# ljishen/bitar

Measured on AMD Instinct MI355X. Metric: GiB/s compress+decompress on 1-GiB Arrow buffer, 1/2/4/8 GPUs; % HBM roofline, higher is better.
Workload: dtype u8; 1 GPU; LZ4 block compress + decompress round trip, 1 GiB per GPU, 64 KiB segments, Silesia-style mix (BASELINE configs[2]); bytes_per_gpu=1073741824, segment_bytes=65536, segments_per_gpu=16384, codec=lz4-block, input_kind=1, parallelism=1 GPU

## Files before the change

### bitar_amd/csrc/compress.hip

```cpp
#include "window_parse.hip.h"

namespace bitar_hip {

namespace cmp {

__device__ __forceinline__ uint32_t lane_sel(uint64_t m, uint32_t a, uint32_t b) {
  uint32_t r;
  __asm__("v_cndmask_b32_e64 %0, %1, %2, %3" : "=v"(r) : "v"(b), "v"(a), "s"(m));
  return r;
}

#ifndef BITAR_LZ4_GATHER
#define BITAR_LZ4_GATHER 3
#endif
#ifndef BITAR_LZ4_OBUF
#define BITAR_LZ4_OBUF 512
#endif
constexpr uint32_t kLz4Obuf = BITAR_LZ4_OBUF;
constexpr uint32_t kSeqCap = 64;
struct Lz4Lds {
#if BITAR_LZ4_GATHER == 3
  uint8_t ring[kLz4Obuf + 16];
#elif BITAR_LZ4_GATHER == 2
  uint8_t ring[kLz4Obuf];
#else
  uint8_t ring[kLz4Obuf + kWave];
#endif
  uint2 seqs[kSeqCap + 1];
  uint32_t marks[kWave + 1];
};

struct Lz4Out : ByteOutT<kLz4Obuf> {
  Lz4Lds* L;
  uint32_t nseq;
  uint32_t last_end;
  uint32_t step_id;

  __device__ __forceinline__ void init(Lz4Lds* lds, GMEM uint8_t* d, uint64_t c) {
    L = lds;
    ring = lds->ring;
    dst = d;
    cap = c;
    op = flushed = 0;
    overflow = false;
    nseq = 0;
    last_end = 0;
    step_id = 0;
    lds->marks[lane_id()] = 0;
    lds_order();
  }
  __device__ __forceinline__ void put_ext(uint32_t v) {
    const uint32_t cnt = v / 255u + 1;
    for (uint32_t k = 0; k < cnt; k += kWave) {
      const uint32_t step = cnt - k < kWave ? cnt - k : kWave;
      if (!room(step)) return;
      const uint32_t t = k + lane_id();
      put(t + 1 < cnt ? 255u : v % 255u, step);
    }
  }
  __device__ __forceinline__ void one(const GMEM uint8_t* in, const InRing& I, uint32_t lit_start,
                                      uint32_t lit_len, uint32_t off, uint32_t mlen) {
    if (overflow) return;
    const uint32_t ml = mlen ? mlen - kMinMatch : 0;
    const uint32_t token = ((lit_len < 15 ? lit_len : 15) << 4) | (ml < 15 ? ml : 15);
    if (!room(1)) return;
    put(token, 1);
    if (lit_len >= 15) put_ext(lit_len - 15);
    if (overflow) return;
    if (lit_len) {
      if ((uint64_t)op + lit_len > cap) { overflow = true; return; }
      if (lit_len <= 256 && lit_start >= I.lo) {
        for (uint32_t k = 0; k < lit_len; k += kWave) {
          const uint32_t step = lit_len - k < kWave ? lit_len - k : kWave;
          room(step);
          lds_order();
          const uint32_t b = I.byte(lit_start + k + (lane_id() < step ? lane_id() : 0u));
          put(b, step);
        }
      } else {
        flush(op, true);
        wave_copy_global(dst + op, in + lit_start, lit_len);
        op += lit_len;
        flushed = op;
      }
    }
    if (!mlen) return;
    if (!room(2)) return;
    put(lane_id() ? off >> 8 : off & 0xFF, 2);
    if (ml >= 15) put_ext(ml - 15);
  }

#if BITAR_LZ4_GATHER == 3
  __device__ __forceinline__ bool bulk(const InRing& I, uint32_t lo, uint32_t hi, uint32_t q,
                                       uint32_t lit_start, uint32_t off, uint32_t mlen) {
    constexpr uint32_t kTrash = kLz4Obuf, kLim = kLz4Obuf - 64;
    const uint32_t lane = lane_id();
    const bool in = (lane >= lo) & (lane < hi);
    const uint32_t lit_len = q - lit_start, ml = mlen - kMinMatch;
    const uint32_t nlx = lit_len >= 15 ? 1u : 0u, nmx = ml >= 15 ? 1u : 0u;
    const uint32_t e = in ? (3u + nlx + nmx + lit_len) | (lit_len << 16) : 0u;
    const uint32_t incl = wave_incl_sum(e);
    const uint32_t total = readlane(incl, kWave - 1) & 0xFFFFu;
// ... 95 lines not shown
      if (op + kWave - flushed > kLz4Obuf - 64) flush(op, false);
      lds_order();
      const uint32_t slot = min(a4 - (R << 2), (uint32_t)kWave << 2);
      *reinterpret_cast<uint32_t*>(reinterpret_cast<uint8_t*>(L->marks) + slot) = mark;
      lds_order();
      const uint32_t mk = L->marks[lane];
      L->marks[lane] = zero;
      const uint64_t S = ballot(mk == u);
      const uint32_t base = before + (uint32_t)(S & 1u);
      const uint64_t S1 = S >> 1;
      const uint32_t idx = __builtin_amdgcn_mbcnt_hi((uint32_t)(S1 >> 32),
                                                     __builtin_amdgcn_mbcnt_lo((uint32_t)S1, 0u));
      before += (uint32_t)__builtin_popcountll(S);
      const int src = (int)((idx << 2) + (base << 2));
      const uint32_t qA = (uint32_t)__builtin_amdgcn_ds_bpermute(src, (int)pA);
      const uint32_t qH = (uint32_t)__builtin_amdgcn_ds_bpermute(src, (int)pH);
      const uint32_t qT = (uint32_t)__builtin_amdgcn_ds_bpermute(src, (int)pT);
      const uint32_t r = u - (qA & 0xFFFFu);
      const uint32_t t = u - (qA >> 16);
      const uint32_t sel = min(min(t, r + 4u), 6u);
      const uint32_t litb = I.ring[(((u << 16) + qH) >> 16) & I.mask];
      const uint32_t hi4 = __builtin_amdgcn_perm(litb, qH, 0x0C040100u);
      const uint32_t b = __builtin_amdgcn_perm(hi4, qT, sel);
      const uint32_t nb = total - R < kWave ? total - R : kWave;
      ring[(rbase + u) & kMask] = (uint8_t)b;
      lds_order();
      op += nb;
      u += kWave;
    }
    return true;
  }
#else
  __device__ __forceinline__ bool bulk(const InRing& I, uint32_t lo, uint32_t hi, uint32_t q,
                                       uint32_t lit_start, uint32_t off, uint32_t mlen) {
    const uint32_t lane = lane_id();
    const bool in = (lane >= lo) & (lane < hi);
    const uint32_t lit_len = q - lit_start, ml = mlen - kMinMatch;
    const uint32_t nlx = lit_len >= 15 ? 1u : 0u, nmx = ml >= 15 ? 1u : 0u;
    const uint32_t e = in ? 3u + nlx + nmx + lit_len : 0u;
    const uint32_t incl = wave_incl_sum(e);
    const uint32_t total = readlane(incl, kWave - 1);
    if ((uint64_t)op + total > cap) return false;
    const uint32_t a = incl - e;
    const uint32_t tok = ((lit_len < 15 ? lit_len : 15) << 4) | (ml < 15 ? ml : 15);
    const uint32_t p0 = a | (lit_len << 16) | (nlx << 25) | (nmx << 26);
    const uint32_t p1 = lit_start | (tok << 16);
    const uint32_t p2 = (off & 0xFFFFu) | (((ml - 15u) & 0xFFu) << 16) | ((lit_len - 15u) << 24);
    for (uint32_t R = 0; R < total; R += kWave) {
      room(kWave);
      step_id += 1;
      const bool st = in & (a - R < kWave);
      lds_order();
      L->marks[st ? a - R : kWave] = (step_id << 8) | (lane + 1);
      lds_order();
      const uint32_t mk = L->marks[lane];
      const uint32_t before = (uint32_t)__builtin_popcountll(ballot(in & (a < R)));
      const uint32_t carry = before ? lo + before : 0u;
      const uint32_t v = (mk >> 8) == step_id ? (mk & 0xFFu) : 0u;
      const uint32_t s1 = max(wave_incl_max(v), carry);
      const int src = (int)((s1 - 1) << 2);
      const uint32_t q0 = (uint32_t)__builtin_amdgcn_ds_bpermute(src, (int)p0);
      const uint32_t q1 = (uint32_t)__builtin_amdgcn_ds_bpermute(src, (int)p1);
      const uint32_t q2 = (uint32_t)__builtin_amdgcn_ds_bpermute(src, (int)p2);
      const uint32_t r = R + lane - (q0 & 0xFFFFu);
      const uint32_t ll = (q0 >> 16) & 511u;
      const uint32_t L0 = 1u + ((q0 >> 25) & 1u), h = L0 + ll;
      const uint32_t litb = I.byte((q1 & 0xFFFFu) + r - L0);
      uint32_t b = r == h + 2 ? (q2 >> 16) & 0xFFu : (q2 >> 8) & 0xFFu;
      b = r == h ? q2 & 0xFFu : b;
      b = r < h ? litb : b;
      b = r < L0 ? q2 >> 24 : b;
      b = r == 0 ? (q1 >> 16) & 0xFFu : b;
      const uint32_t nb = total - R < kWave ? total - R : kWave;
      lds_order();
      ring[lane < nb ? at(op + lane) : kLz4Obuf + lane] = (uint8_t)b;
      lds_order();
      op += nb;
    }
    return true;
  }
#endif

  __device__ __forceinline__ void flush_seqs(const GMEM uint8_t* in, const InRing& I) {
    const uint32_t cnt = nseq;
    nseq = 0;
    if (!cnt || overflow) return;
    const uint32_t lane = lane_id();
    lds_order();
    const uint2 rec = L->seqs[lane < cnt ? lane : kSeqCap];
    const uint32_t q = rec.x & 0xFFFFu, off = (rec.x >> 16) + 1u, mlen = rec.y;
    const uint32_t end = q + mlen;
    const uint32_t prev = wave_shr1(end);
    const uint32_t lit_start = lane == 0 ? last_end : prev;
    const uint32_t lit_len = q - lit_start;
    last_end = readlane(end, cnt - 1);
    const uint64_t live = cnt < kWave ? (1ull << cnt) - 1 : ~0ull;
    uint64_t special = (ballot(lit_len >= 270u) | ballot(mlen >= 270u + kMinMatch) |
                        ballot(lit_start < I.lo)) & live;
    uint32_t lo = 0;
    for (;;) {
      const uint32_t k = special ? (uint32_t)__builtin_ctzll(special) : cnt;
      if (k > lo && !bulk(I, lo, k, q, lit_start, off, mlen)) {
        for (uint32_t j = lo; j < k && !overflow; ++j)
          one(in, I, readlane(lit_start, j), readlane(lit_len, j), readlane(off, j),
              readlane(mlen, j));
      }
      if (k >= cnt || overflow) break;
      one(in, I, readlane(lit_start, k), readlane(lit_len, k), readlane(off, k),
          readlane(mlen, k));
      special &= special - 1;
      lo = k + 1;
    }
  }

  __device__ __forceinline__ void sequence(const GMEM uint8_t* in, const InRing& I,
                                           uint32_t lit_start, uint32_t lit_len, uint32_t off,
                                           uint32_t mlen) {
    flush_seqs(in, I);
    one(in, I, lit_start, lit_len, off, mlen);
  }
  __device__ __forceinline__ uint32_t pending_from(uint32_t anchor, uint32_t) const { return anchor; }

  __device__ __forceinline__ void between(const GMEM uint8_t* in, const InRing& I) {
    if (BITAR_RARE(nseq > kSeqCap - 16)) flush_seqs(in, I);
  }
  __device__ __forceinline__ void window(const GMEM uint8_t*, const InRing&, const Window& W,
                                         uint32_t, uint32_t) {
    if (!W.chain) return;
    const uint64_t chain = W.chain;
    const uint32_t idx = __builtin_amdgcn_mbcnt_hi((uint32_t)(chain >> 32),
                                                   __builtin_amdgcn_mbcnt_lo((uint32_t)chain, nseq));
    const uint32_t lane = lane_id();
    lds_order();
    L->seqs[lane_sel(chain, idx, kSeqCap)] =
        make_uint2((W.x + lane) | (W.dm1 << 16), W.mlen);
    lds_order();
    nseq += (uint32_t)__builtin_popcountll(chain);
  }
};

constexpr uint32_t kBitWords = BITAR_CMP_BITWORDS, kBitMask = kBitWords - 1;

__device__ __forceinline__ uint32_t rev(uint32_t v, uint32_t n) {
  return __builtin_bitreverse32(v) >> (32 - n);
}
__device__ __forceinline__ uint32_t fixed_code(uint32_t s, uint32_t& n) {
  const uint32_t code = s < 144 ? 0x30 + s : s < 256 ? 0x190 + (s - 144) : s < 280 ? s - 256 : 0xC0 + (s - 280);
  n = s < 144 ? 8u : s < 256 ? 9u : s < 280 ? 7u : 8u;
  return __builtin_bitreverse32(code) >> (32 - n);
}
__device__ __forceinline__ uint32_t match_code(uint32_t mlen, uint32_t off, uint32_t& n) {
  const uint32_t v = mlen - 3;
  const uint32_t lev = 29u - __builtin_clz(v | 8u);
  const uint32_t le = mlen == 258 || v < 8 ? 0u : lev;
  const uint32_t lc = mlen == 258 ? 28u : v < 8 ? v : 4 * lev + 4 + ((v >> lev) & 3u);
  const uint32_t lx = v & ((1u << le) - 1);
  const uint32_t d = off - 1;
  const uint32_t dev = 30u - __builtin_clz(d | 4u);
  const uint32_t de = d < 4 ? 0u : dev;
  const uint32_t dc = d < 4 ? d : 2 * dev + 2 + ((d >> dev) & 1u);
  const uint32_t dx = d & ((1u << de) - 1);
  uint32_t ln;
  const uint32_t code = fixed_code(257 + lc, ln);
  n = ln + le + 5 + de;
  return code | (lx << ln) | (rev(dc, 5) << (ln + le)) | (dx << (ln + le + 5));
}

#ifndef BITAR_DFL_BULK
#define BITAR_DFL_BULK 1
#endif
struct DflLds {
  uint2 recs[kSeqCap + 1];
  uint32_t marks[kWave + 1];
};
struct DflOut {
  uint32_t* stage;
  GMEM uint32_t* dst;
  uint64_t cap;
  uint64_t bits;
  uint32_t wflushed;
  bool overflow;

  __device__ __forceinline__ void flush_words(uint32_t upto) {
    const uint32_t lane = lane_id();
    lds_order();
    for (uint32_t w = wflushed + lane; w < upto; w += kWave) {
      dst[w] = stage[w & kBitMask];
      stage[w & kBitMask] = 0;
    }
    lds_order();
    wflushed = upto;
  }
  __device__ __forceinline__ void drain() {
    const uint32_t full = (uint32_t)(bits >> 5);
    if (full != wflushed) flush_words(full);
  }
  __device__ __forceinline__ void put_lanes(uint32_t val, uint32_t nb) {
    if (overflow) return;
    const uint32_t incl = wave_incl_sum(nb);
    const uint32_t total = readlane(incl, 63);
    if ((bits + total + 7) / 8 > cap) { overflow = true; return; }
    const uint64_t bp = bits + incl - nb;
    const uint32_t w = (uint32_t)(bp >> 5), sh = (uint32_t)(bp & 31);
    const uint32_t spill = sh + nb > 32 ? val >> ((32 - sh) & 31) : 0u;
    lds_order();
    if (nb) atomicOr(&stage[w & kBitMask], val << sh);
    if (sh + nb > 32) atomicOr(&stage[(w + 1) & kBitMask], spill);
    lds_order();
    bits += total;
    const uint32_t full = (uint32_t)(bits >> 5);
    if (full - wflushed >= kBitWords - 80) flush_words(full);
  }
  __device__ __forceinline__ void put_one(uint32_t val, uint32_t nb) {
    put_lanes(lane_id() == 0 ? val : 0u, lane_id() == 0 ? nb : 0u);
  }
  __device__ __forceinline__ void literals(const GMEM uint8_t* in, const InRing& I, uint32_t s,
                                           uint32_t n) {
    const uint32_t lane = lane_id();
    const bool ring_ok = s >= I.lo;
    for (uint32_t k = 0; k < n; k += kWave) {
      const uint32_t step = n - k < kWave ? n - k : kWave;
      const uint32_t q = s + k + (lane < step ? lane : 0);
      uint32_t b;
      lds_order();
      if (ring_ok) b = I.byte(q);
      else b = lane < step ? (uint32_t)in[q] : 0u;
      uint32_t nb;
      const uint32_t code = fixed_code(b, nb);
      put_lanes(lane < step ? code : 0u, lane < step ? nb : 0u);
      if (overflow) return;
    }
  }
#if BITAR_DFL_BULK
  DflLds* L;
  uint32_t npend, last_end;

  __device__ __forceinline__ void bulk(const InRing& I, uint32_t lo, uint32_t hi,
                                       uint32_t lit_start, uint32_t ll, uint32_t mv, uint32_t mb) {
    const uint32_t lane = lane_id();
    const bool in = (lane >= lo) & (lane < hi);
    const uint32_t e = in ? ll + 1u : 0u;
    const uint32_t incl = wave_incl_sum(e);
    const uint32_t total = readlane(incl, kWave - 1);
    const uint32_t a = incl - e;
    const uint32_t D = I.in_lo + lit_start - a - 1u;
    const uint32_t pX = ((a + ll + 1u) << 16) | mb;
    const uint32_t a4 = in ? a << 2 : 0x7FFFFF00u;
    const uint32_t mark = a + 1u;
    const uint32_t zero = 0;
    uint32_t u = lane + 1u;
    uint32_t before = lo - 1u;
    for (uint32_t R = 0; R < total && !overflow; R += kWave) {
      lds_order();
      const uint32_t slot = min(a4 - (R << 2), (uint32_t)kWave << 2);
      *reinterpret_cast<uint32_t*>(reinterpret_cast<uint8_t*>(L->marks) + slot) = mark;
      lds_order();
      const uint32_t mk = L->marks[lane];
      L->marks[lane] = zero;
      const uint64_t S = ballot(mk == u);
      const uint32_t base = before + (uint32_t)(S & 1u);
      const uint64_t S1 = S >> 1;
      const uint32_t k = __builtin_amdgcn_mbcnt_hi((uint32_t)(S1 >> 32),
                                                   __builtin_amdgcn_mbcnt_lo((uint32_t)S1, 0u));
      before += (uint32_t)__builtin_popcountll(S);
      const int src = (int)((k << 2) + (base << 2));
      const uint32_t qD = (uint32_t)__builtin_amdgcn_ds_bpermute(src, (int)D);
      const uint32_t qX = (uint32_t)__builtin_amdgcn_ds_bpermute(src, (int)pX);
      const uint32_t qM = (uint32_t)__builtin_amdgcn_ds_bpermute(src, (int)mv);
      const uint32_t b = I.ring[(qD + u) & I.mask];
      uint32_t lb;
      const uint32_t lv = fixed_code(b, lb);
      const bool ism = u == (qX >> 16);
      const bool live = u <= total;
      put_lanes(ism ? qM : lv, live ? (ism ? (qX & 63u) : lb) : 0u);
      u += kWave;
    }
  }
  __device__ __forceinline__ void flush_seqs(const GMEM uint8_t* in, const InRing& I) {
    const uint32_t cnt = npend;
    npend = 0;
    if (!cnt || overflow) return;
    const uint32_t lane = lane_id();
    lds_order();
    const uint2 rec = L->recs[lane < cnt ? lane : kSeqCap];
    const uint32_t q = rec.x & 0xFFFFu, off = (rec.x >> 16) + 1u, mlen = rec.y;
    const uint32_t end = q + mlen;
    const uint32_t prev = wave_shr1(end);
    const uint32_t lit_start = lane == 0 ? last_end : prev;
    const uint32_t ll = q - lit_start;
    last_end = readlane(end, cnt - 1);
    uint32_t mb;
    const uint32_t mv = match_code(lane < cnt ? mlen : 3u, lane < cnt ? off : 1u, mb);
    const uint64_t live = cnt < kWave ? (1ull << cnt) - 1 : ~0ull;
    uint64_t special = ballot(lit_start < I.lo) & ballot(ll != 0u) & live;
    uint32_t lo = 0;
    for (;;) {
      const uint32_t k = special ? (uint32_t)__builtin_ctzll(special) : cnt;
      if (k > lo) bulk(I, lo, k, lit_start, ll, mv, mb);
      if (k >= cnt || overflow) break;
      literals(in, I, readlane(lit_start, k), readlane(ll, k));
      put_one(readlane(mv, k), readlane(mb, k));
      special &= special - 1;
      lo = k + 1;
    }
  }
  __device__ __forceinline__ uint32_t pending_from(uint32_t anchor, uint32_t) const { return anchor; }
  __device__ __forceinline__ void between(const GMEM uint8_t* in, const InRing& I) {
    if (BITAR_RARE(npend > kSeqCap - 16)) flush_seqs(in, I);
  }
  __device__ __forceinline__ void sequence(const GMEM uint8_t* in, const InRing& I, uint32_t s,
                                           uint32_t n, uint32_t, uint32_t) {
    flush_seqs(in, I);
    literals(in, I, s, n);
  }
  __device__ __forceinline__ void window(const GMEM uint8_t*, const InRing&, const Window& W,
// ... 173 lines not shown
```

### bitar_amd/csrc/deflate_dyn.hip

```cpp
#include "huffman.hip.h"
#include "window_parse.hip.h"

namespace bitar_hip {

namespace dyn {

using namespace cmp;

#ifndef BITAR_DYN_VARIANT
#define BITAR_DYN_VARIANT 0
#endif

constexpr uint32_t kPlanBytes = 2048;
constexpr uint32_t kNLit = 286, kNDist = 30, kNCl = 19;
constexpr uint32_t kPlanRecBytes = kNLit + kNDist;

__device__ __forceinline__ uint32_t len_sym(uint32_t mlen, uint32_t& nx, uint32_t& xv) {
  const uint32_t v = mlen - 3;
  const uint32_t lev = 29u - __builtin_clz(v | 8u);
  nx = mlen == 258 || v < 8 ? 0u : lev;
  xv = v & ((1u << nx) - 1);
  return mlen == 258 ? 28u : v < 8 ? v : 4 * lev + 4 + ((v >> lev) & 3u);
}
__device__ __forceinline__ uint32_t dist_sym(uint32_t off, uint32_t& nx, uint32_t& xv) {
// ... 3 lines not shown
  xv = d & ((1u << nx) - 1);
  return d < 4 ? d : 2 * dev + 2 + ((d >> dev) & 1u);
}
__device__ __forceinline__ uint32_t len_extra_bits(uint32_t ls) {
  return ls < 8 || ls == 28 ? 0u : (ls - 4) >> 2;
}
__device__ __forceinline__ uint32_t dist_extra_bits(uint32_t ds) {
  return ds < 4 ? 0u : (ds - 2) >> 1;
}
__constant__ uint8_t kClo[19] = {16, 17, 18, 0, 8, 7, 9, 6, 10, 5, 11, 4, 12, 3, 13, 2, 14, 1, 15};

__device__ __forceinline__ uint32_t fixed_len(uint32_t s) {
  return s < 144 ? 8u : s < 256 ? 9u : s < 280 ? 7u : 8u;
}

[[maybe_unused]] constexpr uint32_t kMaskBytes = 16384;
constexpr uint32_t kPlanWindows = kPlanRecBytes + 1;
constexpr uint32_t kPlanTail = kPlanRecBytes + 2;

constexpr uint32_t kRecBuf = 512, kMaskRing = 32;
struct RecOut : ByteOutT<kRecBuf> {
  uint32_t* lh;
  uint32_t* dh;
  uint4* cst;
  GMEM uint4* cdst;
  uint32_t nwin, cflushed;

  __device__ __forceinline__ void window(const GMEM uint8_t*, const InRing&, const Window& W,
                                         uint32_t, uint32_t n) {
    const uint32_t lane = lane_id();
    const uint32_t q = W.x + lane;
    const bool cl = (W.chain >> lane) & 1;
    const uint32_t pend = wave_incl_max(cl ? q + W.mlen : 0u);
    const bool covered = q < W.pos_in || (!cl && q < pend);
    const bool lit = !cl && !covered && q < n;
    const uint64_t litm = ballot(lit);
    uint32_t lnx, lxv, dnx, dxv;
    const uint32_t ls = len_sym(cl ? W.mlen : 3u, lnx, lxv);
    const uint32_t ds = dist_sym(cl ? W.off() : 1u, dnx, dxv);
    lds_order();
    if (lit) atomicAdd(&lh[W.byte], 1u);
    if (cl) {
      atomicAdd(&lh[257 + ls], 1u);
      atomicAdd(&dh[ds], 1u);
    }
    if (lane == 0)
      cst[nwin & (kMaskRing - 1)] = make_uint4((uint32_t)W.chain, (uint32_t)(W.chain >> 32), (uint32_t)litm,
                                   (uint32_t)(litm >> 32));
    lds_order();
    ++nwin;
    if (overflow || !W.chain) return;
    const uint32_t nm = (uint32_t)__builtin_popcountll(W.chain);
    if (!room(4 * nm)) return;
    const uint32_t rank = (uint32_t)__builtin_popcountll(W.chain & ((1ull << lane) - 1));
    uint32_t* r32 = reinterpret_cast<uint32_t*>(ring);
    lds_order();
    if (cl) r32[at(op + 4 * rank) >> 2] = ls | (lxv << 5) | (ds << 10) | (dxv << 15);
    lds_order();
    op += 4 * nm;
  }
  __device__ __forceinline__ void flush_masks(uint32_t upto) {
    const uint32_t lane = lane_id();
    lds_order();
    for (uint32_t w = cflushed + lane; w < upto; w += kWave) cdst[w] = cst[w & (kMaskRing - 1)];
    cflushed = upto;
  }
  __device__ __forceinline__ void drain() {
    ByteOutT<kRecBuf>::drain();
    flush_masks(nwin);
  }
  __device__ __forceinline__ void sequence(const GMEM uint8_t* in, const InRing& I, uint32_t s,
                                           uint32_t n, uint32_t, uint32_t) {
    const uint32_t lane = lane_id();
    const bool ring_ok = s >= I.lo;
    for (uint32_t k = 0; k < n; k += kWave) {
      const uint32_t step = n - k < kWave ? n - k : kWave;
      const uint32_t q = s + k + (lane < step ? lane : 0);
      lds_order();
      const uint32_t b = ring_ok ? I.byte(q) : (uint32_t)in[q];
      if (lane < step) atomicAdd(&lh[b], 1u);
      lds_order();
    }
  }
  __device__ __forceinline__ void between(const GMEM uint8_t*, const InRing&) {}
  __device__ __forceinline__ uint32_t pending_from(uint32_t, uint32_t emitted) const { return emitted; }
};

#ifndef BITAR_DYN_BULK
#define BITAR_DYN_BULK 1
#endif
#if BITAR_DYN_BULK
constexpr uint32_t kDynCap = 64;
#ifndef BITAR_DYN_OBUF
#define BITAR_DYN_OBUF 512
#endif
constexpr uint32_t kDynObuf = BITAR_DYN_OBUF;
constexpr uint32_t kDynGap = 1024;
__host__ __device__ constexpr uint32_t lit_cap(uint32_t seg) { return (seg + 15u) & ~15u; }
struct DynLds {
  uint8_t ring[kDynObuf];
  uint2 recs[kDynCap + 1];
  uint32_t marks[kWave + 1];
};
struct DynCollect : ByteOutT<kDynObuf> {
  DynLds* L;
  uint32_t* lh;
  uint32_t* dh;
  GMEM uint2* seqs;
  uint32_t nseq, rec_cap, npend;
  uint32_t last_end;
  uint32_t x_seen;

  __device__ __forceinline__ void lit_run(const GMEM uint8_t* in, const InRing& I, uint32_t s,
                                          uint32_t len) {
    const uint32_t lane = lane_id();
    for (uint32_t k = 0; k < len && !overflow; k += kWave) {
      const uint32_t step = len - k < kWave ? len - k : kWave;
      if (!room(step)) return;
      const uint32_t q = s + k + (lane < step ? lane : 0u);
      lds_order();
      const uint32_t b = s + k >= I.lo ? I.byte(q) : (uint32_t)in[q];
      if (lane < step) atomicAdd(&lh[b], 1u);
      put(b, step);
    }
  }
  __device__ __forceinline__ void gather(const InRing& I, uint32_t lo, uint32_t hi,
                                         uint32_t lit_start, uint32_t ll) {
    const uint32_t lane = lane_id();
    const bool ne = (lane >= lo) & (lane < hi) & (ll != 0u);
    const uint32_t e = ne ? ll : 0u;
    const uint32_t incl = wave_incl_sum(e);
    const uint32_t total = readlane(incl, kWave - 1);
    if (!total) return;
    if ((uint64_t)op + total > cap) { overflow = true; return; }
    const uint32_t a = incl - e;
    const uint64_t nem = ballot(ne);
    const uint32_t rank = __builtin_amdgcn_mbcnt_hi((uint32_t)(nem >> 32),
                                                    __builtin_amdgcn_mbcnt_lo((uint32_t)nem, 0u));
    const uint32_t D = I.in_lo + lit_start - a - 1u;
    lds_order();
    uint32_t* tmp = reinterpret_cast<uint32_t*>(L->recs);
    tmp[ne ? rank : kWave] = D;
    lds_order();
    const uint32_t Dc = tmp[lane];
    const uint32_t a4 = ne ? a << 2 : 0x7FFFFF00u;
    const uint32_t mark = a + 1u;
    const uint32_t zero = 0;
    const uint32_t rbase = (uint32_t)(uintptr_t)dst + op - 1u;
    uint32_t u = lane + 1u;
    uint32_t before = 0;
    lds_order();
    for (uint32_t R = 0; R < total; R += kWave) {
      if (op + kWave - flushed > kDynObuf - 64) flush(op, false);
      lds_order();
      const uint32_t slot = min(a4 - (R << 2), (uint32_t)kWave << 2);
      *reinterpret_cast<uint32_t*>(reinterpret_cast<uint8_t*>(L->marks) + slot) = mark;
      lds_order();
      const uint32_t mk = L->marks[lane];
      L->marks[lane] = zero;
      const uint64_t S = ballot(mk == u);
      const uint32_t base = before - 1u + (uint32_t)(S & 1u);
      const uint64_t S1 = S >> 1;
      const uint32_t k = __builtin_amdgcn_mbcnt_hi((uint32_t)(S1 >> 32),
                                                   __builtin_amdgcn_mbcnt_lo((uint32_t)S1, 0u));
      before += (uint32_t)__builtin_popcountll(S);
      const uint32_t d = (uint32_t)__builtin_amdgcn_ds_bpermute((int)((k << 2) + (base << 2)),
                                                                (int)Dc);
      const uint32_t b = I.ring[(d + u) & I.mask];
      const uint32_t nb = total - R < kWave ? total - R : kWave;
      if (lane < nb) atomicAdd(&lh[b], 1u);
      ring[(rbase + u) & kMask] = (uint8_t)b;
      lds_order();
      op += nb;
      u += kWave;
    }
  }
  __device__ __forceinline__ void flush_seqs(const GMEM uint8_t* in, const InRing& I) {
    const uint32_t cnt = npend;
    npend = 0;
    if (overflow) return;
    const uint32_t lane = lane_id();
    if (cnt) {
      lds_order();
      const uint2 rec = L->recs[lane < cnt ? lane : kDynCap];
      const uint32_t q = rec.x & 0xFFFFu, off = (rec.x >> 16) + 1u, mlen = rec.y;
      const uint32_t end = q + mlen;
      const uint32_t prev = wave_shr1(end);
      const uint32_t lit_start = lane == 0 ? last_end : prev;
      const uint32_t ll = q - lit_start;
      last_end = readlane(end, cnt - 1);
      if (nseq + cnt > rec_cap) { overflow = true; return; }
      if (lane < cnt) seqs[nseq + lane] = rec;
      nseq += cnt;
      uint32_t lnx, lxv, dnx, dxv;
      const uint32_t ls = len_sym(lane < cnt ? mlen : 3u, lnx, lxv);
      const uint32_t ds = dist_sym(lane < cnt ? off : 1u, dnx, dxv);
      lds_order();
      if (lane < cnt) {
        atomicAdd(&lh[257 + ls], 1u);
        atomicAdd(&dh[ds], 1u);
      }
      lds_order();
      const uint64_t live = cnt < kWave ? (1ull << cnt) - 1 : ~0ull;
      uint64_t special = ballot(lit_start < I.lo) & ballot(ll != 0u) & live;
      uint32_t lo = 0;
      for (;;) {
        const uint32_t k = special ? (uint32_t)__builtin_ctzll(special) : cnt;
        if (k > lo) gather(I, lo, k, lit_start, ll);
        if (k >= cnt || overflow) break;
        lit_run(in, I, readlane(lit_start, k), readlane(ll, k));
        special &= special - 1;
        lo = k + 1;
      }
    }
    if (x_seen > last_end && !overflow) {
      lit_run(in, I, last_end, x_seen - last_end);
      last_end = x_seen;
    }
  }
  __device__ __forceinline__ void between(const GMEM uint8_t* in, const InRing& I) {
    if (npend > kDynCap - 16 || x_seen > last_end + kDynGap) flush_seqs(in, I);
  }
  __device__ __forceinline__ void sequence(const GMEM uint8_t* in, const InRing& I, uint32_t s,
                                           uint32_t len, uint32_t, uint32_t) {
    x_seen = s + len;
    flush_seqs(in, I);
  }
  __device__ __forceinline__ uint32_t pending_from(uint32_t anchor, uint32_t) const { return anchor; }
  __device__ __forceinline__ void window(const GMEM uint8_t*, const InRing&, const Window& W,
                                         uint32_t, uint32_t n) {
    x_seen = W.x + kWave < n ? W.x + kWave : n;
    if (!W.chain) return;
    const uint64_t chain = W.chain;
    const uint32_t lane = lane_id();
    const uint32_t rank = __builtin_amdgcn_mbcnt_hi((uint32_t)(chain >> 32),
                                                    __builtin_amdgcn_mbcnt_lo((uint32_t)chain, 0u));
    lds_order();
    L->recs[(chain >> lane) & 1u ? npend + rank : kDynCap] =
        make_uint2((W.x + lane) | (W.dm1 << 16), W.mlen);
    lds_order();
    npend += (uint32_t)__builtin_popcountll(chain);
  }
};
#endif

using huf::TreeLds;
using huf::huff_lengths;

__device__ void canon_codes(const uint8_t* lens, uint32_t n, uint32_t* tab) {
  const uint32_t lane = lane_id();
  const uint64_t lt = (1ull << lane) - 1;
  uint32_t cnt[16];
#pragma unroll
  for (int b = 0; b < 16; ++b) cnt[b] = 0;
  lds_order();
  for (uint32_t s0 = 0; s0 < n; s0 += kWave) {
    const uint32_t s = s0 + lane;
    const uint32_t l = s < n ? lens[s] : 0u;
#pragma unroll
    for (int b = 1; b < 16; ++b) cnt[b] += (uint32_t)__builtin_popcountll(ballot(l == (uint32_t)b));
  }
  uint32_t first[16];
  uint32_t code = 0;
  first[0] = 0;
#pragma unroll
  for (int b = 1; b < 16; ++b) {
    code = (code + (b > 1 ? cnt[b - 1] : 0u)) << 1;
    first[b] = code;
    cnt[b - 1] = 0;
  }
  cnt[15] = 0;
  for (uint32_t s0 = 0; s0 < n; s0 += kWave) {
    const uint32_t s = s0 + lane;
    const uint32_t l = s < n ? lens[s] : 0u;
    uint32_t c = 0;
#pragma unroll
    for (int b = 1; b < 16; ++b) {
      const uint64_t m = ballot(l == (uint32_t)b);
      c = l == (uint32_t)b ? first[b] + cnt[b] + (uint32_t)__builtin_popcountll(m & lt) : c;
      cnt[b] += (uint32_t)__builtin_popcountll(m);
    }
    if (s < n) tab[s] = (l ? __builtin_bitreverse32(c) >> (32 - l) : 0u) | (l << 16);
  }
  lds_order();
}

__device__ uint32_t rle_lens(const uint8_t* lens, uint32_t n, uint16_t* out) {
  uint32_t k = 0;
  int prevlen = -1, count = 0, max_count = 7, min_count = 4;
  int nextlen = lens[0];
  if (nextlen == 0) { max_count = 138; min_count = 3; }
  for (uint32_t i = 0; i < n; ++i) {
    const int curlen = nextlen;
    nextlen = i + 1 < n ? (int)lens[i + 1] : 0xFFFF;
    if (++count < max_count && curlen == nextlen) continue;
    if (count < min_count) {
      do { out[k++] = (uint16_t)curlen; } while (--count != 0);
    } else if (curlen != 0) {
      if (curlen != prevlen) { out[k++] = (uint16_t)curlen; --count; }
      out[k++] = (uint16_t)(16 | ((count - 3) << 8));
    } else if (count <= 10) {
      out[k++] = (uint16_t)(17 | ((count - 3) << 8));
// ... 536 lines not shown
```

### bitar_amd/csrc/snappy.hip

```cpp
#include "order.hip.h"
#include "stream_ring.hip.h"
#include "window_parse.hip.h"

namespace bitar_hip {

namespace snp {

__device__ __forceinline__ uint32_t lane_sel(uint64_t m, uint32_t a, uint32_t b) {
  uint32_t r;
  __asm__("v_cndmask_b32_e64 %0, %1, %2, %3" : "=v"(r) : "v"(b), "v"(a), "s"(m));
  return r;
}

__device__ __forceinline__ uint32_t lit_hdr(uint32_t len) {
  return len <= 60u ? 1u : len <= 256u ? 2u : 3u;
}

}

namespace cmp {

constexpr uint32_t kSnapObuf = 512;
constexpr uint32_t kSnapSeqCap = 64;
constexpr uint32_t kSnapBulkLit = 256, kSnapBulkMatch = 64;
// ... 128 lines not shown
      c1r = c1r < hi ? c1r : hi;
      c1r = c1r > c0 ? c1r : c0 + 1u;
      const uint32_t end = readlane(incl, c1r - 1);
      const uint32_t ea = end & 0xFFFFu, el = end >> 16;
      if (op + (ea - ba) - flushed > kLim) flush(op, false);
      lds_order();
      const uint64_t cm = ((c1r < kWave ? 1ull << c1r : 0ull) - 1ull) & ~((1ull << c0) - 1ull);
      ring[snp::lane_sel(cm & l1m, x0, kTrash)] = (uint8_t)h0;
      ring[snp::lane_sel(cm & l2m, x1, kTrash)] = (uint8_t)(lit_len - 1u);
      ring[snp::lane_sel(cm, x2, kTrash)] = (uint8_t)t0;
      ring[snp::lane_sel(cm, x3, kTrash)] = (uint8_t)off;
      ring[snp::lane_sel(cm & c3m, x4, kTrash)] = (uint8_t)(off >> 8);
      for (uint32_t R = bl; R < el; R += kWave) {
        const uint32_t nb = el - R < kWave ? el - R : kWave;
        const uint64_t vm = nb < kWave ? (1ull << nb) - 1ull : ~0ull;
        lds_order();
        const uint32_t slot = min(lp4 - (R << 2), (uint32_t)kWave << 2);
        *reinterpret_cast<uint32_t*>(reinterpret_cast<uint8_t*>(L->marks) + slot) = mark;
        lds_order();
        const uint32_t mk = L->marks[lane];
        L->marks[lane] = zero;
        const uint64_t S = ballot(mk == u) & vm;
        const uint32_t base = before - 1u + (uint32_t)(S & 1u);
        const uint64_t S1 = S >> 1;
        const uint32_t k = __builtin_amdgcn_mbcnt_hi((uint32_t)(S1 >> 32),
                                                     __builtin_amdgcn_mbcnt_lo((uint32_t)S1, 0u));
        before += (uint32_t)__builtin_popcountll(S);
        const uint32_t p = (uint32_t)__builtin_amdgcn_ds_bpermute((int)((k << 2) + (base << 2)),
                                                                  (int)Pc);
        const uint32_t b = I.ring[(p + u) & I.mask];
        ring[snp::lane_sel(vm, ((p >> 16) + u) & kMask, kTrash)] = (uint8_t)b;
        u += nb;
      }
      lds_order();
      op += ea - ba;
      ba = ea;
      bl = el;
      c0 = c1r;
    } while (c0 < hi);
    return true;
  }

  __device__ __forceinline__ void flush_seqs(const GMEM uint8_t* in, const InRing& I) {
    const uint32_t cnt = nseq;
    nseq = 0;
    if (!cnt || overflow) return;
    matched = true;
    const uint32_t lane = lane_id();
    lds_order();
    const uint2 rec = L->seqs[lane < cnt ? lane : kSnapSeqCap];
    const uint32_t q = rec.x & 0xFFFFu, off = (rec.x >> 16) + 1u, mlen = rec.y;
    const uint32_t end = q + mlen;
    const uint32_t prev = wave_shr1(end);
    const uint32_t lit_start = lane == 0 ? last_end : prev;
    const uint32_t lit_len = q - lit_start;
    last_end = readlane(end, cnt - 1);
    const uint64_t live = cnt < kWave ? (1ull << cnt) - 1 : ~0ull;
    uint64_t special = (ballot(lit_len > kSnapBulkLit) | ballot(mlen > kSnapBulkMatch) |
                        ballot(lit_start < I.lo)) & live;
    uint32_t lo = 0;
    for (;;) {
      const uint32_t k = special ? (uint32_t)__builtin_ctzll(special) : cnt;
      if (k > lo && !bulk(I, lo, k, q, lit_start, off, mlen)) {
        for (uint32_t j = lo; j < k && !overflow; ++j)
          one(in, I, readlane(lit_start, j), readlane(lit_len, j), readlane(off, j),
              readlane(mlen, j));
      }
      if (k >= cnt || overflow) break;
      one(in, I, readlane(lit_start, k), readlane(lit_len, k), readlane(off, k),
          readlane(mlen, k));
      special &= special - 1;
      lo = k + 1;
    }
  }

  __device__ __forceinline__ void sequence(const GMEM uint8_t* in, const InRing& I,
                                           uint32_t lit_start, uint32_t lit_len, uint32_t off,
                                           uint32_t mlen) {
    flush_seqs(in, I);
    one(in, I, lit_start, lit_len, off, mlen);
  }
  __device__ __forceinline__ uint32_t pending_from(uint32_t anchor, uint32_t) const { return anchor; }

  __device__ __forceinline__ void between(const GMEM uint8_t* in, const InRing& I) {
    if (BITAR_RARE(nseq > kSnapSeqCap - 16)) flush_seqs(in, I);
  }
  __device__ __forceinline__ void window(const GMEM uint8_t*, const InRing&, const Window& W,
                                         uint32_t, uint32_t) {
    if (!W.chain) return;
    const uint64_t chain = W.chain;
    const uint32_t idx = __builtin_amdgcn_mbcnt_hi((uint32_t)(chain >> 32),
                                                   __builtin_amdgcn_mbcnt_lo((uint32_t)chain, nseq));
    const uint32_t lane = lane_id();
    lds_order();
    L->seqs[snp::lane_sel(chain, idx, kSnapSeqCap)] =
        make_uint2((W.x + lane) | (W.dm1 << 16), W.mlen);
    lds_order();
    nseq += (uint32_t)__builtin_popcountll(chain);
  }
};

}

__global__ __launch_bounds__(64) void snappy_compress_kernel(
    const uint8_t* __restrict__ input, uint64_t n_total, uint32_t seg,
    uint8_t* __restrict__ slab, uint64_t slot_stride, uint8_t* const* __restrict__ dsts,
    uint32_t* __restrict__ sizes, const uint32_t* __restrict__ order) {
  using namespace cmp;
  __shared__ __attribute__((aligned(16))) uint16_t table[(1u << kHashLog) + 8];
  __shared__ __attribute__((aligned(16))) uint8_t inring[kIn + kInPad];
  __shared__ __attribute__((aligned(16))) SnapLds olds;
  const uint32_t i_seg = order ? order[blockIdx.x] : blockIdx.x;
  const uint64_t seg_off = (uint64_t)i_seg * seg;
  if (seg_off >= n_total) return;
  const uint32_t n = (uint32_t)((n_total - seg_off) < seg ? (n_total - seg_off) : seg);
  const GMEM uint8_t* in = global_ptr(input + seg_off);
  SnapOut o;
  o.init(&olds, global_ptr(dsts ? dsts[i_seg] : slab + (uint64_t)i_seg * slot_stride), slot_stride);
  o.preamble(n);
  parse<SnapOut, false, true, kIn, kHashLog, BITAR_CMP_CHAIN>(in, n, global_ptr(input + n_total),
                                                              table, inring, kIn - 1536u,
                                                              0xFFFFFFFFu, o);
  o.flush(o.op, true);
  const uint32_t nb = n < 128u ? 1u : n < 16384u ? 2u : 3u;
  const uint32_t nh = snp::lit_hdr(n);
  const uint32_t stored = nb + nh + n;
  uint32_t size = o.op;
  if (o.overflow || (size >= stored && o.matched)) {
    global_fence_wave();
    const uint32_t lane = lane_id(), m = n - 1u;
    const uint32_t pv = lane == 0 ? (n & 127u) | (nb > 1 ? 128u : 0u)
                        : lane == 1 ? ((n >> 7) & 127u) | (nb > 2 ? 128u : 0u) : n >> 14;
    const uint32_t t = lane - nb;
    const uint32_t hv = t == 0 ? (nh == 1 ? m << 2 : (58u + nh) << 2) : t == 1 ? m & 0xFFu : m >> 8;
    if (lane < nb + nh) o.dst[lane] = (uint8_t)(lane < nb ? pv : hv);
    wave_copy_global(o.dst + nb + nh, in, n);
    size = stored;
  }
  if (lane_id() == 0) sizes[i_seg] = size;
}

namespace snd {

using namespace sr;

constexpr uint32_t kJoinBlock = 65536;
constexpr uint64_t kJoinMaxFragment = 5ull * kJoinBlock;

constexpr uint32_t kBatchIn = 144;
constexpr uint32_t kNextStop = 256;

#define BITAR_SN_LINK                       \
  "s_bitset1_b64 %[ch], %[l]\n"             \
  "v_readlane_b32 %[l], %[nx], %[l]\n"      \
  "s_nop 0\n"
#define BITAR_SN_STEP BITAR_SN_LINK "s_cmp_gt_u32 %[l], 63\n" "s_cbranch_scc1 L_so_%=\n"
#define BITAR_SN_STEP4 BITAR_SN_STEP BITAR_SN_STEP BITAR_SN_STEP BITAR_SN_STEP
__device__ __forceinline__ uint32_t walk_chain(uint32_t nx, uint64_t& chain) {
  uint32_t l = 0;
  __asm__ volatile(
      "L_sc_%=:\n"
      BITAR_SN_STEP4 BITAR_SN_STEP4 BITAR_SN_STEP4 BITAR_SN_STEP BITAR_SN_STEP BITAR_SN_STEP
      BITAR_SN_LINK
      "s_cmp_lt_u32 %[l], 64\n"
      "s_cbranch_scc1 L_sc_%=\n"
      "L_so_%=:\n"
// ... 612 lines not shown
```

### bitar_amd/csrc/window_parse.hip.h

```cpp
#pragma once

#include "wave.hip.h"

namespace bitar_hip {

namespace cmp {

#ifndef BITAR_CMP_HASH_LOG
#define BITAR_CMP_HASH_LOG 10
#endif
#ifndef BITAR_CMP_OBUF
#define BITAR_CMP_OBUF 1024
#endif
#ifndef BITAR_CMP_BITWORDS
#define BITAR_CMP_BITWORDS 256
#endif
constexpr uint32_t kHashLog = BITAR_CMP_HASH_LOG;
constexpr uint32_t kMinMatch = 4;
constexpr uint32_t kLastLiterals = 5;
constexpr uint32_t kMfLimit = 12;
#ifndef BITAR_CMP_RING
#define BITAR_CMP_RING 4096
#endif
constexpr uint32_t kIn = BITAR_CMP_RING, kInMask = kIn - 1;
// ... 535 lines not shown
            }
            const uint64_t stop = ballot(kk >= li || cl < 16);
            if (stop) {
              const uint32_t sl = (uint32_t)__builtin_ctzll(stop);
              const uint32_t ks = k + 16u * sl;
              k = ks >= li ? li : ks + readlane(cl, sl);
              break;
            }
            k += 16u * kWave;
          }
          mlen = k;
          if (lane == l) mlen_v = mlen;
        }
        chain |= 1ull << l;
        e = l + mlen;
        m = e < kWave ? valid & (~0ull << e) : 0ull;
      }
#if BITAR_CMP_CHAIN >= 3
      }
#endif
      if (chain) pos = x + e;
      if constexpr (REP) {
        if (chain) {
          const uint32_t offv = dm1 + 1u;
          const uint32_t n0 = readlane(offv, highbit(chain));
          const uint64_t m1 = chain & ballot(offv != n0);
          const uint32_t o1 = h0 != n0 ? h0 : h1;
          const uint32_t n1 = m1 ? readlane(offv, highbit(m1)) : o1;
          const uint64_t m2 = m1 & ballot(offv != n1);
          const uint32_t o2 = h0 != n0 && h0 != n1 ? h0 : h1 != n0 && h1 != n1 ? h1 : h2;
          const uint32_t n2 = m2 ? readlane(offv, highbit(m2)) : o2;
          h0 = n0;
          h1 = n1;
          h2 = n2;
        }
      }
      Window W;
      W.x = x;
      W.chain = chain;
      W.mlen = mlen_v;
      W.dm1 = dm1;
      W.byte = v.x & 0xFFu;
      W.pos_in = pos_in;
      W.done = emitted;
#ifndef BITAR_CMP_TIMING_NOEMIT
      em.window(in, I, W, anchor, n);
#endif
      if (chain) anchor = pos;
      emitted = pos > x + kWave ? pos : x + kWave;
#if !BITAR_CMP_NOREDO
      uint32_t bk = back;
      __asm__ volatile("" : "+v"(bk));
      if (ballot(bk < p) & actm) {
        bool redo = act && bk < p;
        while (ballot(redo)) {
          lds_order();
          if (redo) table[h] = (uint16_t)p;
          lds_order();
          redo = redo && table[h] < p;
        }
      }
#endif
    };
    uint4 nxt = load_row(1);
    {
      const uint4 r0 = load_row(0);
      lds_order();
      write_row(0, r0);
    }
    F = kRow - s0;
    I.lo = 0;
    lds_order();
    vp = I.bytes16(lane);
    uint32_t next_load = kRow / 2;
    uint32_t g = 0;
    for (uint32_t x = 0; x <= last_start;) {
      if (BITAR_RARE(x >= next_load)) {
        const uint32_t k = next_load / kRow;
        lds_order();
        write_row(k + 1, nxt);
        F = kRow * (k + 2) - s0;
        I.lo = F > RING ? F - RING : 0u;
        em.drain();
        nxt = load_row(k + 2);
        next_load += kRow;
      }
      em.between(in, I);
      if constexpr (SKIP) {
        if (BITAR_RARE(x - g + (kWave - 1) >= kSkipProbe + kWave - 1)) {
          if (pos >= x + kWave) {
            const uint32_t xs = x + ((pos - x) & ~(kWave - 1));
            x = xs < next_load ? xs : next_load;
            lds_order();
            vp = I.bytes16(x + lane);
            continue;
          }
          if (x >= g + kSkipProbe) {
            const uint32_t st = x >= g + kSkipWide ? 4u : 2u;
            lds_order();
            const uint32_t p = x + st * lane;
            const bool act = p <= last_start;
            const uint32_t v = I.dword(p);
            const uint32_t h = hash4<HLOG>(v);
            const uint32_t cand = table[h];
            const uint32_t cv = I.dword(cand);
            const bool hit = act & (cand < p) & (p - cand <= max_dist) & (cv == v);
            if (!ballot(hit)) {
              lds_order();
              table[act ? h : (1u << HLOG)] = (uint16_t)p;
              lds_order();
#if !BITAR_CMP_NOREDO
              bool redo = act && table[h] < p;
              while (ballot(redo)) {
                lds_order();
                if (redo) table[h] = (uint16_t)p;
                lds_order();
                redo = redo && table[h] < p;
              }
#endif
              x += st * kWave;
              continue;
            }
            g = x + kWave * (st - 1) - 127u;
          }
          lds_order();
          vp = I.bytes16(x + lane);
        }
      }
      lds_order();
      window(x);
      if constexpr (SKIP) g = g > pos ? g : pos;
      x += kWave;
    }
  }
  const uint32_t t0 = em.pending_from(anchor, emitted);
  if (t0 < n) em.sequence(in, I, t0, n - t0, 0, 0);
  return t0;
}

}

}
```

### bitar_amd/csrc/zstd_compress.hip

```cpp
#include "huffman.hip.h"
#include "zstd_layout.hip.h"
#include "window_parse.hip.h"

namespace bitar_hip {

namespace zse {

using namespace cmp;

#ifndef BITAR_ZSTD_STOP
#define BITAR_ZSTD_STOP 0
#endif
#define ZSE_PHASE(k)                             \
  if constexpr (BITAR_ZSTD_STOP == (k)) {        \
    if (lane == 0) wrec[zse::kWHanded] = 0u;     \
    return;                                      \
  }

constexpr uint32_t kLLBase[36] = {0,  1,  2,  3,  4,  5,  6,   7,   8,   9,    10,   11,
                                  12, 13, 14, 15, 16, 18, 20,  22,  24,  28,   32,   40,
                                  48, 64, 128, 256, 512, 1024, 2048, 4096, 8192, 16384,
                                  32768, 65536};
constexpr uint8_t kLLBits[36] = {0, 0, 0, 0, 0, 0, 0, 0, 0, 0, 0,  0,  0,  0,  0,  0,  1,  1,
                                 1, 1, 2, 2, 3, 3, 4, 6, 7, 8, 9, 10, 11, 12, 13, 14, 15, 16};
// ... 97 lines not shown
    }
  }
  __device__ __forceinline__ void gather(const InRing& I, uint32_t lo, uint32_t hi,
                                         uint32_t lit_start, uint32_t ll) {
    const uint32_t lane = lane_id();
    const bool ne = (lane >= lo) & (lane < hi) & (ll != 0u);
    const uint32_t e = ne ? ll : 0u;
    const uint32_t incl = wave_incl_sum(e);
    const uint32_t total = readlane(incl, kWave - 1);
    if (!total) return;
    const uint32_t a = incl - e;
    const uint64_t nem = ballot(ne);
    const uint32_t rank = __builtin_amdgcn_mbcnt_hi((uint32_t)(nem >> 32),
                                                    __builtin_amdgcn_mbcnt_lo((uint32_t)nem, 0u));
    const uint32_t D = I.in_lo + lit_start - a - 1u;
    lds_order();
    uint32_t* tmp = reinterpret_cast<uint32_t*>(L->recs);
    tmp[ne ? rank : kWave] = D;
    lds_order();
    const uint32_t Dc = tmp[lane];
    const uint32_t a4 = ne ? a << 2 : 0x7FFFFF00u;
    const uint32_t mark = a + 1u;
    const uint32_t zero = 0;
    const uint32_t rbase = (uint32_t)(uintptr_t)dst + op - 1u;
    uint32_t u = lane + 1u;
    uint32_t before = 0;
    lds_order();
    for (uint32_t R = 0; R < total; R += kWave) {
      if (op + kWave - flushed > kZsObuf - 64) flush(op, false);
      lds_order();
      const uint32_t slot = min(a4 - (R << 2), (uint32_t)kWave << 2);
      *reinterpret_cast<uint32_t*>(reinterpret_cast<uint8_t*>(L->marks) + slot) = mark;
      lds_order();
      const uint32_t mk = L->marks[lane];
      L->marks[lane] = zero;
      const uint64_t S = ballot(mk == u);
      const uint32_t base = before - 1u + (uint32_t)(S & 1u);
      const uint64_t S1 = S >> 1;
      const uint32_t k = __builtin_amdgcn_mbcnt_hi((uint32_t)(S1 >> 32),
                                                   __builtin_amdgcn_mbcnt_lo((uint32_t)S1, 0u));
      before += (uint32_t)__builtin_popcountll(S);
      const uint32_t d = (uint32_t)__builtin_amdgcn_ds_bpermute((int)((k << 2) + (base << 2)),
                                                                (int)Dc);
      const uint32_t b = I.ring[(d + u) & I.mask];
      const uint32_t nb = total - R < kWave ? total - R : kWave;
      ring[(rbase + u) & kMask] = (uint8_t)b;
      lds_order();
      op += nb;
      u += kWave;
    }
  }
  __device__ __forceinline__ void flush_seqs(const GMEM uint8_t* in, const InRing& I) {
    const uint32_t cnt = npend;
    npend = 0;
    if (!cnt) return;
    const uint32_t lane = lane_id();
    lds_order();
    const uint2 rec = L->recs[lane < cnt ? lane : kZsCap];
    const uint32_t q = rec.x & 0xFFFFu, off = (rec.x >> 16) + 1u, mlen = rec.y;
    const uint32_t end = q + mlen;
    const uint32_t prev = wave_shr1(end);
    const uint32_t lit_start = lane == 0 ? last_end : prev;
    const uint32_t ll = q - lit_start;
    last_end = readlane(end, cnt - 1);
    if (lane < cnt) seqs[nseq + lane] = make_uint2(ll | (off << 17), mlen);
    nseq += cnt;
    const uint64_t live = cnt < kWave ? (1ull << cnt) - 1 : ~0ull;
    uint64_t special = ballot(lit_start < I.lo) & ballot(ll != 0u) & live;
    uint32_t lo = 0;
    for (;;) {
      const uint32_t k = special ? (uint32_t)__builtin_ctzll(special) : cnt;
      if (k > lo) gather(I, lo, k, lit_start, ll);
      if (k >= cnt) break;
      literals(in, I, readlane(lit_start, k), readlane(ll, k));
      special &= special - 1;
      lo = k + 1;
    }
  }
  __device__ __forceinline__ void sequence(const GMEM uint8_t* in, const InRing& I, uint32_t s,
                                           uint32_t len, uint32_t, uint32_t) {
    flush_seqs(in, I);
    literals(in, I, s, len);
  }
  __device__ __forceinline__ void between(const GMEM uint8_t* in, const InRing& I) {
    if (npend > kZsCap - 16) flush_seqs(in, I);
  }
  __device__ __forceinline__ uint32_t pending_from(uint32_t anchor, uint32_t) const {
    return anchor;
  }
  __device__ __forceinline__ void window(const GMEM uint8_t*, const InRing&, const Window& W,
                                         uint32_t, uint32_t) {
    if (!W.chain) return;
    const uint64_t chain = W.chain;
    const uint32_t idx = __builtin_amdgcn_mbcnt_hi((uint32_t)(chain >> 32),
                                                   __builtin_amdgcn_mbcnt_lo((uint32_t)chain, npend));
    const uint32_t lane = lane_id();
    lds_order();
    L->recs[(chain >> lane) & 1u ? idx : kZsCap] =
        make_uint2((W.x + lane) | (W.dm1 << 16), W.mlen);
    lds_order();
    npend += (uint32_t)__builtin_popcountll(chain);
  }
};
#else
struct SeqCollect : ByteOut {
  GMEM uint2* seqs;
  uint32_t nseq;

  __device__ __forceinline__ void literals(const GMEM uint8_t* in, const InRing& I, uint32_t s,
                                           uint32_t len) {
    if (!len) return;
    const uint32_t lane = lane_id();
    if (len <= 256 && s >= I.lo) {
      for (uint32_t k = 0; k < len; k += kWave) {
        const uint32_t step = len - k < kWave ? len - k : kWave;
        room(step);
        lds_order();
        const uint32_t b = I.byte(s + k + (lane < step ? lane : 0u));
        put(b, step);
      }
    } else {
      flush(op, true);
      wave_copy_global(dst + op, in + s, len);
      op += len;
      flushed = op;
    }
  }
  __device__ __forceinline__ void sequence(const GMEM uint8_t* in, const InRing& I, uint32_t s,
                                           uint32_t len, uint32_t, uint32_t) {
    literals(in, I, s, len);
  }
  __device__ __forceinline__ void between(const GMEM uint8_t*, const InRing&) {}
  __device__ __forceinline__ uint32_t pending_from(uint32_t, uint32_t emitted) const {
    return emitted;
  }
  __device__ __forceinline__ void window(const GMEM uint8_t* in, const InRing& I,
                                         const Window& W, uint32_t anchor, uint32_t n) {
    if (W.done < W.x) literals(in, I, W.done, W.x - W.done);
    const uint32_t lane = lane_id();
    const uint32_t q = W.x + lane;
    const bool cl = (W.chain >> lane) & 1;
    const uint32_t end_incl = wave_incl_max(cl ? q + W.mlen : 0u);
    const uint32_t end_excl = wave_shr1(end_incl);
    const uint32_t lit_start = max(anchor, cl ? end_excl : end_incl);
    const uint32_t ll = q - lit_start;
    const bool lit = !cl && q >= W.pos_in && q >= end_incl && q < n;
    const uint64_t litm = ballot(lit);
    const uint32_t nl = (uint32_t)__builtin_popcountll(litm);
    if (nl) {
      room(nl);
      const uint32_t li = __builtin_amdgcn_mbcnt_hi((uint32_t)(litm >> 32),
                                                    __builtin_amdgcn_mbcnt_lo((uint32_t)litm, 0u));
      lds_order();
      ring[lit ? at(op + li) : kObuf + lane] = (uint8_t)W.byte;
      lds_order();
      op += nl;
    }
    if (W.chain) {
      const uint32_t si = __builtin_amdgcn_mbcnt_hi((uint32_t)(W.chain >> 32),
                                                    __builtin_amdgcn_mbcnt_lo((uint32_t)W.chain, 0u));
      if (cl) seqs[nseq + si] = make_uint2(ll | (W.off() << 17), W.mlen);
      nseq += (uint32_t)__builtin_popcountll(W.chain);
    }
  }
};
#endif

__device__ __forceinline__ uint32_t rep_scan(uint32_t ll, uint32_t o, bool act, uint32_t cnt,
                                             uint32_t& c0r, uint32_t& c1r, uint32_t& c2r) {
  const uint32_t lane = lane_id();
  const uint32_t so = wave_shr1(o);
  const uint32_t oprev = lane == 0 ? c0r : so;
  const bool same = !act || (ll != 0 && o == oprev);
  const uint32_t mj = wave_incl_max(same ? 0u : lane + 1);
  const uint32_t p1 = bpermute(oprev, mj ? mj - 1 : 0u);
  const uint32_t r1a = mj ? p1 : c1r;
  const uint32_t s1 = wave_shr1(r1a);
  const uint32_t r1b = lane == 0 ? c1r : s1;
  const bool ev = !same && o != r1b;
  const uint32_t mk = wave_incl_max(ev ? lane + 1 : 0u);
  const uint32_t p2 = bpermute(r1b, mk ? mk - 1 : 0u);
  const uint32_t r2a = mk ? p2 : c2r;
  const uint32_t s2 = wave_shr1(r2a);
  const uint32_t r2b = lane == 0 ? c2r : s2;
  uint32_t ov;
  if (ll) ov = o == oprev ? 1u : o == r1b ? 2u : o == r2b ? 3u : o + 3u;
  else ov = o == r1b ? 1u : o == r2b ? 2u : o == oprev - 1u ? 3u : o + 3u;
  c0r = readlane(o, cnt - 1);
  c1r = readlane(r1a, cnt - 1);
  c2r = readlane(r2a, cnt - 1);
  return ov;
}

constexpr uint32_t kTabLL = 0, kTabOF = 512, kTabML = 768, kTabDummy = 1280;

struct EntLds {
  uint32_t hist[256];
  uint8_t len[256];
  uint8_t w[256];
  uint8_t desc[192];
  uint8_t tmp[256];
  int16_t norm[64];
  uint32_t u[16];
  uint32_t wk[32];
  uint32_t sh[3][64];
  union {
    huf::TreeLds T;
    struct {
      uint16_t tabs[kTabDummy + 1];
      uint32_t tr[3][64];
      uint8_t sym_at[512];
      uint16_t nxt[64];
    };
  };
// ... 1116 lines not shown
```

Before: 263.3 GiB/s.

## Speculatively stream long LZ4 literal runs to output during row parsing

Adds a speculative path to the LZ4 emitter. When a long run with no matches (past a threshold) is seen while rows are being parsed, literal bytes are written straight to their predicted final output offset with 16-byte vector stores, row by row. When the closing sequence arrives, only the header and length bytes are emitted, so the tail is not copied again. A new sequence cancels the speculation with a fence, which adds per-row bookkeeping and a risk of wasted stores on that path.

```diff
diff --git a/bitar_amd/csrc/compress.hip b/bitar_amd/csrc/compress.hip
--- a/bitar_amd/csrc/compress.hip
+++ b/bitar_amd/csrc/compress.hip
@@ -18,6 +18,15 @@
 #endif
 constexpr uint32_t kLz4Obuf = BITAR_LZ4_OBUF;
 constexpr uint32_t kSeqCap = 64;
+#ifndef BITAR_LZ4_SPEC_T
+#define BITAR_LZ4_SPEC_T 1024
+#endif
+#ifndef BITAR_LZ4_SPEC_PRE
+#define BITAR_LZ4_SPEC_PRE 128
+#endif
+constexpr uint32_t kSpecT = BITAR_LZ4_SPEC_T, kSpecPre = BITAR_LZ4_SPEC_PRE;
+static_assert(kSpecT >= 16 && kSpecT <= 1280, "tail-run threshold: see above");
+constexpr uint32_t kSpec = 0x80000000u;
 struct Lz4Lds {
 #if BITAR_LZ4_GATHER == 3
   uint8_t ring[kLz4Obuf + 16];
@@ -279,9 +288,10 @@
 #endif
 
   __device__ __forceinline__ void flush_seqs(const GMEM uint8_t* in, const InRing& I) {
-    const uint32_t cnt = nseq;
+    const uint32_t cnt = here(nseq & ~kSpec);
     nseq = 0;
     if (!cnt || overflow) return;
+    if (BITAR_RARE(last_end & kSpec)) spec_drop();
     const uint32_t lane = lane_id();
     lds_order();
     const uint2 rec = L->seqs[lane < cnt ? lane : kSeqCap];
@@ -314,7 +324,73 @@
                                            uint32_t lit_start, uint32_t lit_len, uint32_t off,
                                            uint32_t mlen) {
     flush_seqs(in, I);
+    if (last_end == (lit_start | kSpec) && !overflow) {
+      const uint32_t n = lit_start + lit_len;
+      const uint32_t delta = spec_delta(n);
+      if (room(1)) put(0xF0u, 1);
+      put_ext(lit_len - 15u);
+      flush(op, true);
+      const uint32_t d = spec_block(delta, n);
+      lds_order();
+      if (lane_id() < n - d) dst[delta + d + lane_id()] = (uint8_t)I.byte(d + lane_id());
+      op += lit_len;
+      flushed = op;
+      return;
+    }
     one(in, I, lit_start, lit_len, off, mlen);
+  }
+
+  __device__ __forceinline__ uint32_t spec_delta(uint32_t nn) const {
+    const uint32_t a = last_end & ~kSpec;
+    return here(op + 2u + (nn - a - 15u) / 255u - a);
+  }
+  __device__ __forceinline__ uint32_t spec_block(uint32_t delta, uint32_t q) const {
+    return q - (((uint32_t)(uintptr_t)dst + delta + q) & 15u);
+  }
+  __device__ __forceinline__ void spec_store(const InRing& I, uint32_t delta, uint32_t from,
+                                             uint32_t to) {
+    const uint32_t nb = to > from ? (to - from) >> 4 : 0u;
+    uint32_t lane = lane_id();
+    __asm__ volatile("" : "+v"(lane));
+    lds_order();
+    for (uint32_t b = lane; b < nb; b += kWave) {
+      const uint32_t q = from + 16u * b;
+      *reinterpret_cast<GMEM uint4*>(dst + (delta + q)) = I.bytes16(q);
+    }
+  }
+  __device__ __forceinline__ void spec_drop() {
+    last_end &= ~kSpec;
+    global_fence_wave();
+  }
+  __device__ __forceinline__ uint32_t here(uint32_t v) const {
+    __asm__ volatile("" : "+s"(v));
+    return v;
+  }
+  __device__ __forceinline__ void row(const GMEM uint8_t*, const InRing& I, uint32_t anchor,
+                                      uint32_t x, uint32_t F_old, uint32_t F, uint32_t n) {
+    const uint32_t nn = here(n);
+    if (last_end & kSpec) {
+      if (last_end == (anchor | kSpec)) {
+        const uint32_t delta = spec_delta(nn);
+        spec_store(I, delta, spec_block(delta, F_old < nn ? F_old : nn), F < nn ? F : nn);
+        return;
+      }
+      spec_drop();
+    }
+    if (x < anchor + kSpecPre || overflow) return;
+    if (nseq) {
+      nseq |= kSpec;
+      return;
+    }
+    if (x < anchor + kSpecT || anchor < I.lo) return;
+    const uint32_t len = nn - anchor;
+    if ((uint64_t)op + 2u + (len - 15u) / 255u + len > cap) return;
+    last_end |= kSpec;
+    const uint32_t delta = spec_delta(nn);
+    const uint32_t head = (16u - (((uint32_t)(uintptr_t)dst + delta + anchor) & 15u)) & 15u;
+    lds_order();
+    if (lane_id() < head) dst[delta + anchor + lane_id()] = (uint8_t)I.byte(anchor + lane_id());
+    spec_store(I, delta, anchor + head, F < nn ? F : nn);
   }
   __device__ __forceinline__ uint32_t pending_from(uint32_t anchor, uint32_t) const { return anchor; }
 
@@ -428,6 +504,8 @@
       if (overflow) return;
     }
   }
+  __device__ __forceinline__ void row(const GMEM uint8_t*, const InRing&, uint32_t, uint32_t, uint32_t,
+                                      uint32_t, uint32_t) {}
 #if BITAR_DFL_BULK
   DflLds* L;
   uint32_t npend, last_end;
diff --git a/bitar_amd/csrc/deflate_dyn.hip b/bitar_amd/csrc/deflate_dyn.hip
--- a/bitar_amd/csrc/deflate_dyn.hip
+++ b/bitar_amd/csrc/deflate_dyn.hip
@@ -109,6 +109,8 @@
       lds_order();
     }
   }
+  __device__ __forceinline__ void row(const GMEM uint8_t*, const InRing&, uint32_t, uint32_t, uint32_t,
+                                      uint32_t, uint32_t) {}
   __device__ __forceinline__ void between(const GMEM uint8_t*, const InRing&) {}
   __device__ __forceinline__ uint32_t pending_from(uint32_t, uint32_t emitted) const { return emitted; }
 };
@@ -245,6 +247,8 @@
       last_end = x_seen;
     }
   }
+  __device__ __forceinline__ void row(const GMEM uint8_t*, const InRing&, uint32_t, uint32_t, uint32_t,
+                                      uint32_t, uint32_t) {}
   __device__ __forceinline__ void between(const GMEM uint8_t* in, const InRing& I) {
     if (npend > kDynCap - 16 || x_seen > last_end + kDynGap) flush_seqs(in, I);
   }
diff --git a/bitar_amd/csrc/snappy.hip b/bitar_amd/csrc/snappy.hip
--- a/bitar_amd/csrc/snappy.hip
+++ b/bitar_amd/csrc/snappy.hip
@@ -234,6 +234,8 @@
   }
   __device__ __forceinline__ uint32_t pending_from(uint32_t anchor, uint32_t) const { return anchor; }
 
+  __device__ __forceinline__ void row(const GMEM uint8_t*, const InRing&, uint32_t, uint32_t, uint32_t,
+                                      uint32_t, uint32_t) {}
   __device__ __forceinline__ void between(const GMEM uint8_t* in, const InRing& I) {
     if (BITAR_RARE(nseq > kSnapSeqCap - 16)) flush_seqs(in, I);
   }
diff --git a/bitar_amd/csrc/window_parse.hip.h b/bitar_amd/csrc/window_parse.hip.h
--- a/bitar_amd/csrc/window_parse.hip.h
+++ b/bitar_amd/csrc/window_parse.hip.h
@@ -641,6 +641,7 @@
         F = kRow * (k + 2) - s0;
         I.lo = F > RING ? F - RING : 0u;
         em.drain();
+        em.row(in, I, anchor, x, F - kRow, F, n);
         nxt = load_row(k + 2);
         next_load += kRow;
       }
diff --git a/bitar_amd/csrc/zstd_compress.hip b/bitar_amd/csrc/zstd_compress.hip
--- a/bitar_amd/csrc/zstd_compress.hip
+++ b/bitar_amd/csrc/zstd_compress.hip
@@ -203,6 +203,8 @@
     flush_seqs(in, I);
     literals(in, I, s, len);
   }
+  __device__ __forceinline__ void row(const GMEM uint8_t*, const InRing&, uint32_t, uint32_t, uint32_t,
+                                      uint32_t, uint32_t) {}
   __device__ __forceinline__ void between(const GMEM uint8_t* in, const InRing& I) {
     if (npend > kZsCap - 16) flush_seqs(in, I);
   }
@@ -251,6 +253,8 @@
                                            uint32_t len, uint32_t, uint32_t) {
     literals(in, I, s, len);
   }
+  __device__ __forceinline__ void row(const GMEM uint8_t*, const InRing&, uint32_t, uint32_t, uint32_t,
+                                      uint32_t, uint32_t) {}
   __device__ __forceinline__ void between(const GMEM uint8_t*, const InRing&) {}
   __device__ __forceinline__ uint32_t pending_from(uint32_t, uint32_t emitted) const {
     return emitted;
```

Measured after the change: 262.9 GiB/s. Within noise of the previous version (-0.1%).
